# cserteGT3/RANSAC.jl

Hardware: NVIDIA B200
Metric: candidate_point_evals_per_s (higher is better)
Workload: dtype f32

## Files before the change

### ransac.jl_b200/csrc/rsc_eval.cuh

```cuda
#pragma once
#include "rsc_common.cuh"

namespace rsc {

__host__ __device__ constexpr float kappa(int type) {
  return type == RSC_PLANE ? 8.f : type == RSC_SPHERE ? 16.f : type == RSC_CYLINDER ? 16.f : 20.f;
}

__host__ __device__ constexpr float kappa_in(int type) {
  return type == RSC_PLANE ? 1.f : type == RSC_SPHERE ? 3.f : type == RSC_CYLINDER ? 3.f : 4.f;
}

__host__ __device__ inline int col_type(const rsc_cand& c) {
  if (c.type != RSC_CONE) return c.type;
  return cos(0.5 * c.p[6]) >= 0.5 ? RSC_CONE : kConeWide;
}

__device__ __forceinline__ float fmax_nan(float a, float b) {
  float r;
  asm("max.NaN.f32 %0, %1, %2;" : "=f"(r) : "f"(a), "f"(b));
  return r;
}
__device__ __forceinline__ float rsqrt_fast(float a) {
  float r;
// ... 66 lines not shown
    float wn = fmaf(wx, nx, fmaf(wy, ny, wz * nz));
    float an = fmaf(r[4], nx, fmaf(r[5], ny, r[6] * nz));
    float t1 = fmaf(r[0], an, r[9]);
    float cw = r[10] * wn;
    float nt = fmaf(rho, t1, -cw);
    return fmax_nan(e, nt);
  } else {
    float vx = fmaf(r[0], px, r[1]), vy = fmaf(r[0], py, r[2]), vz = fmaf(r[0], pz, r[3]);
    float h = fmaf(r[4], vx, fmaf(r[5], vy, r[6] * vz));
    float wx = fmaf(-r[4], h, vx), wy = fmaf(-r[5], h, vy), wz = fmaf(-r[6], h, vz);
    float ww = fmaf(wx, wx, fmaf(wy, wy, wz * wz));
    float rho = ww * rsqrt_fast(ww);
    float d = fmaf(h, r[7], -rho);
    float e = fabsf(d) + r[8];
    float wn = fmaf(wx, nx, fmaf(wy, ny, wz * nz));
    float an = fmaf(r[4], nx, fmaf(r[5], ny, r[6] * nz));
    float t1 = fmaf(r[7], an, r[9]);
    float nt = fmaf(rho, t1, -wn);
    return fmax_nan(e, nt);
  }
}

__device__ __forceinline__ float2 bc2(float s) { return make_float2(s, s); }
__device__ __forceinline__ float2 neg2(float2 a) { return make_float2(-a.x, -a.y); }
__device__ __forceinline__ float2 abs2(float2 a) { return make_float2(fabsf(a.x), fabsf(a.y)); }
__device__ __forceinline__ float2 fma2(float2 a, float2 b, float2 c) { return __ffma2_rn(a, b, c); }
__device__ __forceinline__ float2 mul2(float2 a, float2 b) { return __fmul2_rn(a, b); }
__device__ __forceinline__ float2 add2(float2 a, float2 b) { return __fadd2_rn(a, b); }
__device__ __forceinline__ float2 rsqrt2(float2 a) { return make_float2(rsqrt_fast(a.x), rsqrt_fast(a.y)); }
__device__ __forceinline__ float2 max2_nan(float2 a, float2 b) {
  return make_float2(fmax_nan(a.x, b.x), fmax_nan(a.y, b.y));
}

template <int T>
__device__ __forceinline__ float2 eval2_terms(const float2* r, float px, float py, float pz, float nx, float ny,
                                              float nz, float eps, float cosa, float2* nt_out) {
  const float2 X = bc2(px), Y = bc2(py), Z = bc2(pz), NX = bc2(nx), NY = bc2(ny), NZ = bc2(nz);
  if constexpr (T == RSC_PLANE) {
    const float2 d = fma2(r[0], X, fma2(r[1], Y, fma2(r[2], Z, r[3])));
    const float2 e = add2(abs2(d), bc2(-eps));
    const float2 nt = fma2(r[4], NX, fma2(r[5], NY, fma2(r[6], NZ, bc2(cosa))));
    *nt_out = nt;
    return e;
  } else if constexpr (T == RSC_SPHERE) {
    const float2 vx = fma2(r[0], X, r[1]), vy = fma2(r[0], Y, r[2]), vz = fma2(r[0], Z, r[3]);
    const float2 vv = fma2(vx, vx, fma2(vy, vy, mul2(vz, vz)));
    const float2 d = fma2(vv, rsqrt2(vv), r[4]);
    const float2 e = add2(abs2(d), bc2(-eps));
    const float2 s = fma2(vx, NX, fma2(vy, NY, fma2(vz, NZ, r[5])));
    const float2 nt = fma2(bc2(cosa), d, neg2(s));
    *nt_out = nt;
    return e;
  } else if constexpr (T == RSC_CYLINDER) {
    const float2 vx = fma2(r[0], X, r[1]), vy = fma2(r[0], Y, r[2]), vz = fma2(r[0], Z, r[3]);
    const float2 h = fma2(r[4], vx, fma2(r[5], vy, mul2(r[6], vz)));
    const float2 wx = fma2(neg2(r[4]), h, vx), wy = fma2(neg2(r[5]), h, vy), wz = fma2(neg2(r[6]), h, vz);
    const float2 ww = fma2(wx, wx, fma2(wy, wy, mul2(wz, wz)));
    const float2 d = fma2(ww, rsqrt2(ww), r[7]);
    const float2 e = add2(abs2(d), bc2(-eps));
    const float2 wn = fma2(wx, NX, fma2(wy, NY, fma2(wz, NZ, r[8])));
    const float2 nt = fma2(bc2(cosa), d, neg2(wn));
    *nt_out = nt;
    return e;
  } else if constexpr (T == kConeWide) {
    const float2 vx = fma2(r[0], X, r[1]), vy = fma2(r[0], Y, r[2]), vz = fma2(r[0], Z, r[3]);
    const float2 h = fma2(r[4], vx, fma2(r[5], vy, mul2(r[6], vz)));
    const float2 wx = fma2(neg2(r[4]), h, vx), wy = fma2(neg2(r[5]), h, vy), wz = fma2(neg2(r[6]), h, vz);
    const float2 ww = fma2(wx, wx, fma2(wy, wy, mul2(wz, wz)));
    const float2 rho = mul2(ww, rsqrt2(ww));
    const float2 d = fma2(neg2(rho), r[7], h);
    const float2 e = add2(abs2(d), r[8]);
    const float2 wn = fma2(wx, NX, fma2(wy, NY, mul2(wz, NZ)));
    const float2 an = fma2(r[4], NX, fma2(r[5], NY, mul2(r[6], NZ)));
    const float2 t1 = fma2(r[0], an, r[9]);
    const float2 cw = mul2(r[10], wn);
    const float2 nt = fma2(rho, t1, neg2(cw));
    *nt_out = nt;
    return e;
  } else {
    const float2 vx = fma2(r[0], X, r[1]), vy = fma2(r[0], Y, r[2]), vz = fma2(r[0], Z, r[3]);
    const float2 h = fma2(r[4], vx, fma2(r[5], vy, mul2(r[6], vz)));
    const float2 wx = fma2(neg2(r[4]), h, vx), wy = fma2(neg2(r[5]), h, vy), wz = fma2(neg2(r[6]), h, vz);
    const float2 ww = fma2(wx, wx, fma2(wy, wy, mul2(wz, wz)));
    const float2 rho = mul2(ww, rsqrt2(ww));
    const float2 d = fma2(h, r[7], neg2(rho));
    const float2 e = add2(abs2(d), r[8]);
    const float2 wn = fma2(wx, NX, fma2(wy, NY, mul2(wz, NZ)));
    const float2 an = fma2(r[4], NX, fma2(r[5], NY, mul2(r[6], NZ)));
    const float2 t1 = fma2(r[7], an, r[9]);
    const float2 nt = fma2(rho, t1, neg2(wn));
    *nt_out = nt;
    return e;
  }
}

template <int T>
__device__ __forceinline__ float2 eval2(const float2* r, float px, float py, float pz, float nx, float ny,
                                        float nz, float eps, float cosa) {
  float2 nt;
  const float2 e = eval2_terms<T>(r, px, py, pz, nx, ny, nz, eps, cosa, &nt);
  return max2_nan(e, nt);
}

template <int T>
__device__ __forceinline__ void eval2x4(const float2* r, const float* px, const float* py, const float* pz, const float* nx,
                                        const float* ny, const float* nz, float eps, float cosa, float2* m) {
#define RSC_Q for (int q = 0; q < 4; ++q)
  if constexpr (T == RSC_PLANE) {
    float2 d[4], nt[4];
#pragma unroll
    RSC_Q d[q] = fma2(r[2], bc2(pz[q]), r[3]);
#pragma unroll
    RSC_Q d[q] = fma2(r[1], bc2(py[q]), d[q]);
#pragma unroll
    RSC_Q d[q] = fma2(r[0], bc2(px[q]), d[q]);
#pragma unroll
    RSC_Q nt[q] = fma2(r[6], bc2(nz[q]), bc2(cosa));
#pragma unroll
    RSC_Q nt[q] = fma2(r[5], bc2(ny[q]), nt[q]);
#pragma unroll
    RSC_Q nt[q] = fma2(r[4], bc2(nx[q]), nt[q]);
#pragma unroll
    RSC_Q d[q] = add2(abs2(d[q]), bc2(-eps));
#pragma unroll
    RSC_Q m[q] = max2_nan(d[q], nt[q]);
  } else {
// ... 257 lines not shown
```

### ransac.jl_b200/csrc/rsc_score.cu

```cuda
#include <math.h>
#include <stdlib.h>

#include "rsc_eval.cuh"
#include "rsc_exact.cuh"

namespace rsc {

struct GroupTask {
  uint32_t cand;
  uint32_t group;
  uint32_t word;
  uint32_t slot_type;
};

struct ScoreArgs {
  PointSet ps;
  Thresh th;
  const float* rec;
  const int32_t* orig;
  const BlockTab* tab;
  int32_t cslots;
  int32_t subs_per_chunk;
  int32_t nsubs;
  int32_t* counts_valid;
  int32_t* counts_enabled;
  uint32_t* masks;
  GroupTask* wl;
  uint32_t* wl_count;
  uint32_t wl_cap;
};

constexpr int kSub = 128;
constexpr int kStages = 2;
constexpr int kSubFloats = 6 * kSub;
// ... 2 lines not shown
__device__ __forceinline__ uint32_t smem_u32(const void* p) { return (uint32_t)__cvta_generic_to_shared(p); }
__device__ __forceinline__ void mbar_init(uint64_t* bar, uint32_t count) {
  asm volatile("mbarrier.init.shared::cta.b64 [%0], %1;" ::"r"(smem_u32(bar)), "r"(count));
}
__device__ __forceinline__ void mbar_expect_tx(uint64_t* bar, uint32_t bytes) {
  asm volatile("mbarrier.arrive.expect_tx.shared::cta.b64 _, [%0], %1;" ::"r"(smem_u32(bar)), "r"(bytes) : "memory");
}
__device__ __forceinline__ void mbar_wait(uint64_t* bar, uint32_t parity) {
  asm volatile(
      "{\n"
      ".reg .pred p;\n"
      "WAIT_%=:\n"
      "mbarrier.try_wait.parity.shared::cta.b64 p, [%0], %1;\n"
      "@p bra DONE_%=;\n"
      "bra WAIT_%=;\n"
      "DONE_%=:\n"
      "}\n" ::"r"(smem_u32(bar)),
      "r"(parity)
      : "memory");
}
__device__ __forceinline__ void bulk_g2s(void* dst, const void* src, uint32_t bytes, uint64_t* bar) {
  asm volatile("cp.async.bulk.shared::cluster.global.mbarrier::complete_tx::bytes [%0], [%1], %2, [%3];" ::"r"(
                   smem_u32(dst)),
               "l"(src), "r"(bytes), "r"(smem_u32(bar))
               : "memory");
}

__device__ __forceinline__ void issue_subtile(const float* src, int64_t stride, float* stage, uint64_t* bar) {
  mbar_expect_tx(bar, kSubBytes);
#pragma unroll
  for (int f = 0; f < 6; ++f) bulk_g2s(stage + f * kSub, src + f * stride, kSub * 4, bar);
}

template <int T, int K, int U, bool MASKS>
__device__ __forceinline__ void score_body(const ScoreArgs& a, int slot0, float* wstage, uint64_t* wbar) {
  constexpr int NR = RecN<T>::n;
  constexpr bool kPacked = (K % 2 == 0) && U < 5;
  constexpr int KP = kPacked ? K / 2 : 1;
  constexpr bool kOrderJQ = (U == 3);
  float r[kPacked ? 1 : K][NR];
  float2 r2[KP][NR];
  float band[K];
  int cnte[K], cntv[K];
  const int tid = threadIdx.x, lane = tid & 31;
  const float* recp = a.rec + slot0 + tid;
#pragma unroll
  for (int k = 0; k < K; ++k) {
#pragma unroll
    for (int f = 0; f < NR; ++f) {
      const float v = recp[(size_t)f * a.cslots + k * kThreads];
      if constexpr (kPacked) {
        if (k & 1)
          r2[k / 2][f].y = v;
        else
          r2[k / 2][f].x = v;
      } else {
        r[k][f] = v;
      }
    }
    band[k] = recp[(size_t)kBandField * a.cslots + k * kThreads];
    cnte[k] = 0;
    cntv[k] = 0;
  }
  constexpr int PT = public_type(T);
  const float eps = a.th.eps[PT], cosa = a.th.cosa[PT];
  const bool honour = (a.th.honour_enabled >> PT) & 1u;

  const int sub0 = blockIdx.y * a.subs_per_chunk;
  const int nsub = min(a.subs_per_chunk, a.nsubs - sub0);
  const uint32_t* enp = a.ps.enabled + (size_t)sub0 * (kSub / 32);
  const uint32_t* vap = a.ps.valid + (size_t)sub0 * (kSub / 32);
  uint32_t* maskp = MASKS ? a.masks + (size_t)sub0 * (kSub / 32) * a.cslots + slot0 + tid : nullptr;
  const int64_t stride = a.ps.y - a.ps.x;
  const float* src0 = a.ps.x + (int64_t)sub0 * kSub;
  if (lane == 0) {
#pragma unroll
    for (int s = 0; s < kStages; ++s)
      if (s < nsub) issue_subtile(src0 + s * kSub, stride, wstage + s * kSubFloats, wbar + s);
  }

  auto body4 = [&](const float* gp, uint32_t (&mask)[K], float (&mabs)[K]) {
    const float4 X = *reinterpret_cast<const float4*>(gp);
    const float4 Y = *reinterpret_cast<const float4*>(gp + kSub);
    const float4 Z = *reinterpret_cast<const float4*>(gp + 2 * kSub);
    const float4 U4 = *reinterpret_cast<const float4*>(gp + 3 * kSub);
    const float4 V = *reinterpret_cast<const float4*>(gp + 4 * kSub);
    const float4 W = *reinterpret_cast<const float4*>(gp + 5 * kSub);
    const float px[4] = {X.x, X.y, X.z, X.w}, py[4] = {Y.x, Y.y, Y.z, Y.w}, pz[4] = {Z.x, Z.y, Z.z, Z.w};
    const float nx[4] = {U4.x, U4.y, U4.z, U4.w}, ny[4] = {V.x, V.y, V.z, V.w}, nz[4] = {W.x, W.y, W.z, W.w};
    if constexpr (kPacked && U == 4) {
#pragma unroll
      for (int j = 0; j < KP; ++j) {
        float2 m[4];
        eval2x4<T>(r2[j], px, py, pz, nx, ny, nz, eps, cosa, m);
#pragma unroll
        for (int q = 0; q < 4; ++q) {
          mask[2 * j] = __funnelshift_l(__float_as_uint(m[q].x), mask[2 * j], 1);
          mask[2 * j + 1] = __funnelshift_l(__float_as_uint(m[q].y), mask[2 * j + 1], 1);
          mabs[2 * j] = fmin_nan(mabs[2 * j], fabsf(m[q].x));
          mabs[2 * j + 1] = fmin_nan(mabs[2 * j + 1], fabsf(m[q].y));
        }
      }
      return;
    }
    if constexpr (kPacked && kOrderJQ) {
#pragma unroll
      for (int j = 0; j < KP; ++j) {
        float2 m[4];
#pragma unroll
        for (int q = 0; q < 4; ++q) m[q] = eval2<T>(r2[j], px[q], py[q], pz[q], nx[q], ny[q], nz[q], eps, cosa);
#pragma unroll
        for (int q = 0; q < 4; ++q) {
          mask[2 * j] = __funnelshift_l(__float_as_uint(m[q].x), mask[2 * j], 1);
          mask[2 * j + 1] = __funnelshift_l(__float_as_uint(m[q].y), mask[2 * j + 1], 1);
          mabs[2 * j] = fmin_nan(mabs[2 * j], fabsf(m[q].x));
          mabs[2 * j + 1] = fmin_nan(mabs[2 * j + 1], fabsf(m[q].y));
        }
      }
      return;
    }
    if constexpr (!kPacked && U == 6) {
#pragma unroll
      for (int k = 0; k < K; ++k) {
        float m[4];
#pragma unroll
        for (int q = 0; q < 4; ++q) m[q] = eval<T>(r[k], px[q], py[q], pz[q], nx[q], ny[q], nz[q], eps, cosa);
#pragma unroll
        for (int q = 0; q < 4; ++q) {
          mask[k] = __funnelshift_l(__float_as_uint(m[q]), mask[k], 1);
          mabs[k] = fmin_nan(mabs[k], fabsf(m[q]));
        }
      }
      return;
    }
#pragma unroll
    for (int q = 0; q < 4; ++q) {
      if constexpr (kPacked) {
// ... 31 lines not shown
    if constexpr (MASKS) {
      const uint32_t gate = honour ? en : va;
#pragma unroll
      for (int k = 0; k < K; ++k) maskp[(size_t)gi * a.cslots + k * kThreads] = __brev(mask[k]) & gate;
    }
    if (amb && va) {
      const int64_t gw = (int64_t)sub0 * (kSub / 32) + gi;
#pragma unroll
      for (int k = 0; k < K; ++k) {
        if (mabs[k] > band[k]) continue;
        const int slot = slot0 + k * kThreads + tid;
        const int o = a.orig[slot];
        if (o < 0) continue;
        const uint32_t pos = atomicAdd(a.wl_count, 1u);
        if (pos < a.wl_cap) a.wl[pos] = GroupTask{(uint32_t)o, (uint32_t)gw, __brev(mask[k]), (uint32_t)slot | ((uint32_t)T << 28)};
      }
    }
  };

  for (int it = 0; it < nsub; ++it) {
    const int st = it % kStages;
    mbar_wait(wbar + st, (it / kStages) & 1);
    const float* sx = wstage + st * kSubFloats;
#pragma unroll 1
    for (int g = 0; g < kSub / 32; ++g) {
      uint32_t mask[K];
      float mabs[K];
#pragma unroll
      for (int k = 0; k < K; ++k) {
        mask[k] = 0u;
        mabs[k] = __int_as_float(0x7f800000);
      }
      const float* gx = sx + g * 32;
#pragma unroll(U >= 3 ? 1 : U)
      for (int i4 = 0; i4 < 32; i4 += 4) body4(gx + i4, mask, mabs);
      const int gi = it * (kSub / 32) + g;
      epilogue(mask, mabs, gi, __ldg(enp + gi), __ldg(vap + gi));
    }
    __syncwarp();
    if (lane == 0 && it + kStages < nsub) issue_subtile(src0 + (it + kStages) * kSub, stride, wstage + st * kSubFloats, wbar + st);
  }
#pragma unroll
  for (int k = 0; k < K; ++k) {
    const int o = a.orig[slot0 + k * kThreads + tid];
    if (o >= 0) {
      if (cnte[k]) atomicAdd(a.counts_enabled + o, cnte[k]);
      if (!honour && cntv[k]) atomicAdd(a.counts_valid + o, cntv[k]);
    }
  }
}

template <int T, int K, int MINB, int U, bool MASKS>
__global__ void __launch_bounds__(kThreads, MINB) score_kernel(const __grid_constant__ ScoreArgs a) {
  __shared__ __align__(128) float stages[kThreads / 32][kStages * kSubFloats];
  __shared__ __align__(8) uint64_t bars[kThreads / 32][kStages];
  const BlockTab bt = a.tab[blockIdx.x];
  if (bt.type != T) return;
  const int warp = threadIdx.x >> 5;
  if ((threadIdx.x & 31) == 0) {
#pragma unroll
    for (int s = 0; s < kStages; ++s) mbar_init(&bars[warp][s], 1);
    asm volatile("fence.mbarrier_init.release.cluster;" ::: "memory");
  }
  __syncwarp();
  score_body<T, K, U, MASKS>(a, bt.slot0, stages[warp], bars[warp]);
}

template <int K, int MINB, bool MASKS>
__global__ void __launch_bounds__(kThreads, MINB) score_kernel_any(const __grid_constant__ ScoreArgs a) {
  __shared__ __align__(128) float stages[kThreads / 32][kStages * kSubFloats];
  __shared__ __align__(8) uint64_t bars[kThreads / 32][kStages];
  const BlockTab bt = a.tab[blockIdx.x];
  if (bt.type < 0) return;
  const int warp = threadIdx.x >> 5;
  if ((threadIdx.x & 31) == 0) {
#pragma unroll
    for (int s = 0; s < kStages; ++s) mbar_init(&bars[warp][s], 1);
    asm volatile("fence.mbarrier_init.release.cluster;" ::: "memory");
  }
  __syncwarp();
  switch (bt.type) {
    case RSC_PLANE:
      score_body<RSC_PLANE, K, 1, MASKS>(a, bt.slot0, stages[warp], bars[warp]);
      break;
    case RSC_SPHERE:
      score_body<RSC_SPHERE, K, 1, MASKS>(a, bt.slot0, stages[warp], bars[warp]);
      break;
    case RSC_CYLINDER:
      score_body<RSC_CYLINDER, K, 1, MASKS>(a, bt.slot0, stages[warp], bars[warp]);
      break;
    case RSC_CONE:
      score_body<RSC_CONE, K, 1, MASKS>(a, bt.slot0, stages[warp], bars[warp]);
      break;
    default:
      score_body<kConeWide, K, 1, MASKS>(a, bt.slot0, stages[warp], bars[warp]);
      break;
  }
}
// ... 77 lines not shown
    const bool used = pr.cand_bit >> 31;
    const rsc_cand c = cands[cand];
    ex::ConeTrig tr{1.0, 0.0};
    if (c.type == RSC_CONE) {
      if (trig) {
        tr = trig[cand];
      } else {
        tr.ct = cos(-c.p[6] / 2);
        tr.st = sin(-c.p[6] / 2);
      }
    }
    const uint32_t pt = pr.point;
    ex::V3 P, N;
    ex::point64(a.ps, pt, &P, &N);
    const bool ok = ex::compat(c, tr, a.th, P, N);
    if (ok != used) apply_flip(a, cand, c.type, slot_of[cand], pt, ok);
  }
}

__global__ void select_counts_kernel(const rsc_cand* __restrict__ cands, int C,
                                     const int32_t* __restrict__ cv, const int32_t* __restrict__ ce,
                                     uint32_t honour_enabled, int32_t* __restrict__ out) {
  const int i = blockIdx.x * blockDim.x + threadIdx.x;
  if (i >= C) return;
  const int t = cands[i].type;
  const bool honour = (t >= 0 && t < RSC_NTYPES) ? ((honour_enabled >> t) & 1u) : true;
  out[i] = honour ? ce[i] : cv[i];
}

struct ColSlots {
  int v[kColTypes];
};

__global__ void __launch_bounds__(1024) compile_kernel(const rsc_cand* __restrict__ cands, int C, const Thresh th,
                                                       const ColSlots spcs, int cslots,
                                                       int ncols, float pmax, float nmax,
                                                       const uint32_t* __restrict__ d_bounds,
                                                       float* __restrict__ rec, int32_t* __restrict__ orig,
                                                       int32_t* __restrict__ slot_of,
                                                       BlockTab* __restrict__ tab) {
  __shared__ int cnt[kColTypes], off[kColTypes], run[kColTypes], tot[kColTypes];
  __shared__ int wcnt[kColTypes][32], woff[kColTypes][32];
  const int tid = threadIdx.x, lane = tid & 31, warp = tid >> 5;
  if (d_bounds) {
    pmax = sqrtf(__uint_as_float(d_bounds[0])) * 1.000001f;
    nmax = sqrtf(__uint_as_float(d_bounds[1])) * 1.000001f;
  }
  if (tid < kColTypes) {
    cnt[tid] = 0;
    run[tid] = 0;
  }
  __syncthreads();
  for (int i = tid; i < C; i += blockDim.x) {
    const int t = cands[i].type;
    if (t >= 0 && t < RSC_NTYPES) atomicAdd(&cnt[col_type(cands[i])], 1);
  }
  __syncthreads();
  if (tid == 0) {
    const int order[kColTypes] = {kConeWide, RSC_CONE, RSC_CYLINDER, RSC_SPHERE, RSC_PLANE};
    int s = 0, col = 0;
    for (int oi = 0; oi < kColTypes; ++oi) {
      const int t = order[oi];
      off[t] = s;
      const int spc = spcs.v[t];
      const int nb = (cnt[t] + spc - 1) / spc;
      for (int b = 0; b < nb && col < ncols; ++b) tab[col++] = BlockTab{t, s + b * spc};
      s += nb * spc;
    }
    for (; col < ncols; ++col) tab[col] = BlockTab{-1, 0};
  }
  __syncthreads();
  for (int base = 0; base < C; base += blockDim.x) {
    const int i = base + tid;
    int t = -1;
    if (i < C) {
      t = cands[i].type;
      t = (t < 0 || t >= RSC_NTYPES) ? -1 : col_type(cands[i]);
    }
    int myrank = 0;
#pragma unroll
    for (int tt = 0; tt < kColTypes; ++tt) {
      const unsigned b = __ballot_sync(0xffffffffu, t == tt);
      if (t == tt) myrank = __popc(b & ((1u << lane) - 1u));
      if (lane == 0) wcnt[tt][warp] = __popc(b);
    }
    __syncthreads();
    if (warp == 0) {
#pragma unroll
      for (int tt = 0; tt < kColTypes; ++tt) {
        const int v = wcnt[tt][lane];
        int inc = v;
#pragma unroll
        for (int d = 1; d < 32; d <<= 1) {
          const int o = __shfl_up_sync(0xffffffffu, inc, d);
          if (lane >= d) inc += o;
        }
        woff[tt][lane] = inc - v;
        if (lane == 31) tot[tt] = inc;
      }
    }
    __syncthreads();
    if (i < C) {
      if (t >= 0) {
        const int slot = off[t] + run[t] + woff[t][warp] + myrank;
        float r[kRecFields];
        compile_record(cands[i], t, th, pmax, nmax, r);
#pragma unroll
        for (int f = 0; f < kRecFields; ++f) rec[(size_t)f * cslots + slot] = r[f];
        orig[slot] = i;
        slot_of[i] = slot;
      } else {
        slot_of[i] = -1;
      }
    }
    __syncthreads();
    if (tid < kColTypes) run[tid] += tot[tid];
    __syncthreads();
  }
  for (int t = 0; t < kColTypes; ++t) {
    const int n = cnt[t];
    if (n == 0) continue;
    const int spc = spcs.v[t];
    const int padded = ((n + spc - 1) / spc) * spc;
    const int src = off[t] + n - 1;
    for (int s = n + tid; s < padded; s += blockDim.x) {
      const int dst = off[t] + s;
#pragma unroll
      for (int f = 0; f < kRecFields; ++f) rec[(size_t)f * cslots + dst] = rec[(size_t)f * cslots + src];
      orig[dst] = -1;
    }
  }
}

__global__ void __launch_bounds__(1024) masks_transpose_kernel(const uint32_t* __restrict__ gm,
                                                               const int32_t* __restrict__ slot_of,
                                                               int C, int cslots, int64_t words,
                                                               uint32_t* __restrict__ out) {
  __shared__ uint32_t t[32][33];
  const int c0 = blockIdx.x * 32;
  const int64_t g0 = (int64_t)blockIdx.y * 32;
  {
    const int c = c0 + threadIdx.x;
    const int64_t g = g0 + threadIdx.y;
    uint32_t v = 0;
    if (c < C && g < words) {
      const int s = slot_of[c];
      if (s >= 0) v = gm[(size_t)g * cslots + s];
    }
    t[threadIdx.y][threadIdx.x] = v;
  }
  __syncthreads();
  {
    const int c = c0 + threadIdx.y;
    const int64_t g = g0 + threadIdx.x;
    if (c < C && g < words) out[(size_t)c * words + g] = t[threadIdx.x][threadIdx.y];
  }
}

Thresh make_thresh(const rsc_params* p) {
  Thresh th;
  for (int t = 0; t < RSC_NTYPES; ++t) {
    th.eps_d[t] = p->eps[t];
    th.cosa_d[t] = cos(p->alpha[t]);
    th.eps[t] = (float)th.eps_d[t];
    th.cosa[t] = (float)th.cosa_d[t];
  }
  th.honour_enabled = 0xFu;
  if (p->compat_flags & RSC_COMPAT_SPHERE_IGNORES_ENABLED) th.honour_enabled &= ~(1u << RSC_SPHERE);
  return th;
}

using ScoreFn = void (*)(const ScoreArgs);
struct Tiling {
  int K, minb, U;
  ScoreFn fn[kColTypes];
  ScoreFn fn_masks[kColTypes];
};
#define RSC_TILING(K, MINB, U)                                                                          \
  Tiling {                                                                                              \
    K, MINB, U,                                                                                         \
        {score_kernel<RSC_PLANE, K, MINB, U, false>, score_kernel<RSC_SPHERE, K, MINB, U, false>,       \
         score_kernel<RSC_CYLINDER, K, MINB, U, false>, score_kernel<RSC_CONE, K, MINB, U, false>,      \
         score_kernel<kConeWide, K, MINB, U, false>},                                                   \
    {                                                                                                   \
      score_kernel<RSC_PLANE, K, MINB, U, true>, score_kernel<RSC_SPHERE, K, MINB, U, true>,            \
          score_kernel<RSC_CYLINDER, K, MINB, U, true>, score_kernel<RSC_CONE, K, MINB, U, true>,       \
          score_kernel<kConeWide, K, MINB, U, true>                                                     \
    }                                                                                                   \
  }
#ifdef RSC_EXP_K
static const Tiling kTilings[] = {RSC_TILING(1, 4, 1), RSC_TILING(RSC_EXP_K, RSC_EXP_MINB, RSC_EXP_U)};
#else
static const Tiling kTilings[] = {
    RSC_TILING(1, 4, 1), RSC_TILING(2, 4, 1), RSC_TILING(4, 3, 1), RSC_TILING(4, 4, 1), RSC_TILING(8, 2, 1), RSC_TILING(4, 4, 3), RSC_TILING(4, 3, 3),
    RSC_TILING(4, 4, 5), RSC_TILING(4, 3, 5), RSC_TILING(4, 4, 6), RSC_TILING(4, 3, 6), RSC_TILING(8, 2, 5),
};
#endif
static const Tiling* find_tiling(int K, int minb, int U) {
  for (const Tiling& t : kTilings)
    if (t.K == K && t.minb == minb && t.U == U) return &t;
  return nullptr;
}

static int cap_k(int C) { return C >= 3072 ? 8 : (C >= 768 ? 2 : 1); }

static const Tiling* pick_tiling(int type, int C) {
  static const char* names[kColTypes] = {"RSC_CFG_PLANE", "RSC_CFG_SPHERE", "RSC_CFG_CYLINDER", "RSC_CFG_CONE", "RSC_CFG_CONE"};
  static const int dflt[kColTypes][3] = {{4, 4, 3}, {4, 3, 3}, {4, 3, 3}, {4, 3, 3}, {4, 3, 3}};
  int K = dflt[type][0], minb = dflt[type][1], U = dflt[type][2];
  if (const char* e = getenv(names[type])) {
    int a = 0, b = 0, c = 0;
    if (sscanf(e, "%d,%d,%d", &a, &b, &c) == 3 && find_tiling(a, b, c)) K = a, minb = b, U = c;
  }
  const int kc = cap_k(C);
  if (K > kc) {
    K = kc;
    minb = 4, U = 1;
  }
  return find_tiling(K, minb, U);
}

// ... 35 lines not shown
    return RSC_OK;
  }
  if (ps.n_pad >= ((int64_t)1 << 32)) return fail(ctx, RSC_E_ARG, "point set too large for one shard (>= 2^32)");
  {
    const int64_t sd = ps.y - ps.x;
    if (ps.z - ps.y != sd || ps.nx - ps.z != sd || ps.ny - ps.nx != sd || ps.nz - ps.ny != sd)
      return fail(ctx, RSC_E_ARG, "score: the six SoA rows of the point set must be equally spaced");
  }
  const SlotLayout L = slot_layout(C);
  const int ncols = L.ncols, cslots = L.cslots;
  ctx->last_cslots = cslots;
  const int nsubs = (int)(ps.n_pad / kSub);
  const int64_t groups = ps.n_pad / 32;

  RSC_CUDA(ctx, ctx->rec.ensure((size_t)kRecFields * cslots * sizeof(float)));
  RSC_CUDA(ctx, ctx->orig.ensure((size_t)cslots * sizeof(int32_t)));
  RSC_CUDA(ctx, ctx->slot_of.ensure((size_t)C * sizeof(int32_t)));
  RSC_CUDA(ctx, ctx->blktab.ensure((size_t)ncols * sizeof(BlockTab)));
  RSC_CUDA(ctx, ctx->counts.ensure((size_t)2 * C * sizeof(int32_t)));
  RSC_CUDA(ctx, ctx->worklist.ensure(ctx->wl_cap * sizeof(GroupTask)));
  RSC_CUDA(ctx, ctx->wl_count.ensure(16));
  if (want_masks) RSC_CUDA(ctx, ctx->masks_gm.ensure((size_t)groups * cslots * sizeof(uint32_t)));

  int32_t* cv = d_counts_valid ? d_counts_valid : ctx->counts.as<int32_t>();
  int32_t* ce = d_counts_enabled ? d_counts_enabled : ctx->counts.as<int32_t>() + C;
  if (!accumulate) {
    RSC_CUDA(ctx, cudaMemsetAsync(cv, 0, (size_t)C * sizeof(int32_t), st));
    RSC_CUDA(ctx, cudaMemsetAsync(ce, 0, (size_t)C * sizeof(int32_t), st));
  }
  RSC_CUDA(ctx, ctx->pairs.ensure(ctx->wl_cap * 8));
  RSC_CUDA(ctx, cudaMemsetAsync(ctx->wl_count.p, 0, 2 * sizeof(uint32_t), st));

  if (cloud->exact() && !ps.xyz64) return fail(ctx, RSC_E_STATE, "score: a point set of an exact cloud lacks its float64 coordinates");
  Thresh thx = th;
  thx.exact_in = cloud->exact();
  compile_kernel<<<1, 1024, 0, st>>>(d_cands, C, thx, L.spcs, cslots, ncols, cloud->pmax, cloud->nmax, d_bounds,
                                     ctx->rec.as<float>(), ctx->orig.as<int32_t>(),
                                     ctx->slot_of.as<int32_t>(), ctx->blktab.as<BlockTab>());
  RSC_CUDA(ctx, cudaGetLastError());

  ScoreArgs a;
  a.ps = ps;
  a.th = thx;
  a.rec = ctx->rec.as<float>();
  a.orig = ctx->orig.as<int32_t>();
  a.tab = ctx->blktab.as<BlockTab>();
  a.cslots = cslots;
  a.nsubs = nsubs;
  a.counts_valid = cv;
  a.counts_enabled = ce;
  a.masks = want_masks ? ctx->masks_gm.as<uint32_t>() : nullptr;
  a.wl = ctx->worklist.as<GroupTask>();
  a.wl_count = ctx->wl_count.as<uint32_t>();
  a.wl_cap = (uint32_t)ctx->wl_cap;

  const int waves = getenv("RSC_WAVES") ? atoi(getenv("RSC_WAVES")) : 32;
  const int est_cols = (C + kThreads * 4 - 1) / (kThreads * 4);
  const long target = (long)ctx->sm_count * 4 * waves;
  long chunks = (target + est_cols - 1) / est_cols;
  if (chunks > nsubs) chunks = nsubs;
  if (chunks < 1) chunks = 1;
  if (chunks > 65535) chunks = 65535;
  a.subs_per_chunk = (int)((nsubs + chunks - 1) / chunks);
  chunks = (nsubs + a.subs_per_chunk - 1) / a.subs_per_chunk;
  dim3 grid((unsigned)ncols, (unsigned)chunks);
  static const double fork_min = getenv("RSC_FORK_MIN") ? atof(getenv("RSC_FORK_MIN")) : 1e9;
  const bool fork = (double)C * (double)ps.n_pad >= fork_min && !getenv("RSC_NOFORK");

  RSC_CUDA(ctx, cudaEventRecord(ctx->evk0, st));
  const int K0 = L.til[0]->K;
  bool uniform_k = K0 <= 2;
  for (int t = 1; t < kColTypes; ++t) uniform_k = uniform_k && L.til[t]->K == K0;
  if (!fork && uniform_k && !getenv("RSC_NOFUSE")) {
    if (K0 == 1) {
      if (want_masks)
        score_kernel_any<1, 4, true><<<grid, kThreads, 0, st>>>(a);
      else
        score_kernel_any<1, 4, false><<<grid, kThreads, 0, st>>>(a);
    } else {
      if (want_masks)
        score_kernel_any<2, 4, true><<<grid, kThreads, 0, st>>>(a);
      else
        score_kernel_any<2, 4, false><<<grid, kThreads, 0, st>>>(a);
    }
    RSC_CUDA(ctx, cudaGetLastError());
  } else {
    if (fork) RSC_CUDA(ctx, cudaEventRecord(ctx->ev_fork, st));
    const int order[kColTypes] = {RSC_CONE, kConeWide, RSC_CYLINDER, RSC_SPHERE, RSC_PLANE};
    for (int oi = 0; oi < kColTypes; ++oi) {
      const int t = order[oi];
      cudaStream_t s = st;
      if (fork && oi > 0) {
        s = ctx->sfork[oi - 1];
        RSC_CUDA(ctx, cudaStreamWaitEvent(s, ctx->ev_fork, 0));
      }
      (want_masks ? L.til[t]->fn_masks[t] : L.til[t]->fn[t])<<<grid, kThreads, 0, s>>>(a);
      RSC_CUDA(ctx, cudaGetLastError());
      if (fork && oi > 0) {
        RSC_CUDA(ctx, cudaEventRecord(ctx->ev_join[oi - 1], s));
        RSC_CUDA(ctx, cudaStreamWaitEvent(st, ctx->ev_join[oi - 1], 0));
      }
    }
  }
  RSC_CUDA(ctx, cudaGetLastError());
  RSC_CUDA(ctx, cudaEventRecord(ctx->evk1, st));
  ctx->stats.score_launches += 1;
  ctx->stats.evals += (int64_t)C * ps.n;
  ctx->stats.cands_scored += C;

  fixup_scan_kernel<<<ctx->sm_count * 8, 256, 0, st>>>(a, d_cands, ctx->slot_of.as<int32_t>(), ctx->pairs.as<AmbPair>(),
                                                       ctx->wl_count.as<uint32_t>() + 1, (uint32_t)ctx->wl_cap);
  RSC_CUDA(ctx, cudaGetLastError());
  fixup_pair_kernel<<<ctx->sm_count * 4, 256, 0, st>>>(a, d_cands, reinterpret_cast<const ex::ConeTrig*>(d_trig),
                                                       ctx->slot_of.as<int32_t>(), ctx->pairs.as<AmbPair>(),
                                                       ctx->wl_count.as<uint32_t>() + 1, (uint32_t)ctx->wl_cap);
  RSC_CUDA(ctx, cudaGetLastError());
  if (d_counts_policy) {
    select_counts_kernel<<<(C + 255) / 256, 256, 0, st>>>(d_cands, C, cv, ce, th.honour_enabled, d_counts_policy);
    RSC_CUDA(ctx, cudaGetLastError());
  }
  return RSC_OK;
}

__global__ void audit_compile_kernel(const rsc_cand* __restrict__ cands, int C, const Thresh th, float pmax, float nmax,
                                     float* __restrict__ rec , int32_t* __restrict__ cols) {
  const int i = blockIdx.x * blockDim.x + threadIdx.x;
  if (i >= C) return;
  const int col = (cands[i].type < 0 || cands[i].type >= RSC_NTYPES) ? RSC_PLANE : col_type(cands[i]);
  float r[kRecFields];
// ... 78 lines not shown
```

Baseline: 1578.

## Skip normal-angle term when distance rejects whole warp, sort candidates spatially

```diff
diff --git a/ransac.jl_b200/csrc/rsc_eval.cuh b/ransac.jl_b200/csrc/rsc_eval.cuh
--- a/ransac.jl_b200/csrc/rsc_eval.cuh
+++ b/ransac.jl_b200/csrc/rsc_eval.cuh
@@ -122,66 +122,72 @@
   return make_float2(fmax_nan(a.x, b.x), fmax_nan(a.y, b.y));
 }
 
-template <int T>
-__device__ __forceinline__ float2 eval2_terms(const float2* r, float px, float py, float pz, float nx, float ny,
-                                              float nz, float eps, float cosa, float2* nt_out) {
-  const float2 X = bc2(px), Y = bc2(py), Z = bc2(pz), NX = bc2(nx), NY = bc2(ny), NZ = bc2(nz);
+struct Mid2 {
+  float2 x, y, z, s;
+};
+
+template <int T>
+__device__ __forceinline__ float2 eval2_dist(const float2* r, float px, float py, float pz, float eps, Mid2* md) {
+  const float2 X = bc2(px), Y = bc2(py), Z = bc2(pz);
   if constexpr (T == RSC_PLANE) {
     const float2 d = fma2(r[0], X, fma2(r[1], Y, fma2(r[2], Z, r[3])));
-    const float2 e = add2(abs2(d), bc2(-eps));
-    const float2 nt = fma2(r[4], NX, fma2(r[5], NY, fma2(r[6], NZ, bc2(cosa))));
-    *nt_out = nt;
-    return e;
+    return add2(abs2(d), bc2(-eps));
   } else if constexpr (T == RSC_SPHERE) {
     const float2 vx = fma2(r[0], X, r[1]), vy = fma2(r[0], Y, r[2]), vz = fma2(r[0], Z, r[3]);
     const float2 vv = fma2(vx, vx, fma2(vy, vy, mul2(vz, vz)));
     const float2 d = fma2(vv, rsqrt2(vv), r[4]);
-    const float2 e = add2(abs2(d), bc2(-eps));
-    const float2 s = fma2(vx, NX, fma2(vy, NY, fma2(vz, NZ, r[5])));
-    const float2 nt = fma2(bc2(cosa), d, neg2(s));
-    *nt_out = nt;
-    return e;
-  } else if constexpr (T == RSC_CYLINDER) {
-    const float2 vx = fma2(r[0], X, r[1]), vy = fma2(r[0], Y, r[2]), vz = fma2(r[0], Z, r[3]);
-    const float2 h = fma2(r[4], vx, fma2(r[5], vy, mul2(r[6], vz)));
-    const float2 wx = fma2(neg2(r[4]), h, vx), wy = fma2(neg2(r[5]), h, vy), wz = fma2(neg2(r[6]), h, vz);
-    const float2 ww = fma2(wx, wx, fma2(wy, wy, mul2(wz, wz)));
-    const float2 d = fma2(ww, rsqrt2(ww), r[7]);
-    const float2 e = add2(abs2(d), bc2(-eps));
-    const float2 wn = fma2(wx, NX, fma2(wy, NY, fma2(wz, NZ, r[8])));
-    const float2 nt = fma2(bc2(cosa), d, neg2(wn));
-    *nt_out = nt;
-    return e;
-  } else if constexpr (T == kConeWide) {
-    const float2 vx = fma2(r[0], X, r[1]), vy = fma2(r[0], Y, r[2]), vz = fma2(r[0], Z, r[3]);
-    const float2 h = fma2(r[4], vx, fma2(r[5], vy, mul2(r[6], vz)));
-    const float2 wx = fma2(neg2(r[4]), h, vx), wy = fma2(neg2(r[5]), h, vy), wz = fma2(neg2(r[6]), h, vz);
-    const float2 ww = fma2(wx, wx, fma2(wy, wy, mul2(wz, wz)));
-    const float2 rho = mul2(ww, rsqrt2(ww));
-    const float2 d = fma2(neg2(rho), r[7], h);
-    const float2 e = add2(abs2(d), r[8]);
-    const float2 wn = fma2(wx, NX, fma2(wy, NY, mul2(wz, NZ)));
-    const float2 an = fma2(r[4], NX, fma2(r[5], NY, mul2(r[6], NZ)));
-    const float2 t1 = fma2(r[0], an, r[9]);
-    const float2 cw = mul2(r[10], wn);
-    const float2 nt = fma2(rho, t1, neg2(cw));
-    *nt_out = nt;
-    return e;
+    *md = Mid2{vx, vy, vz, d};
+    return add2(abs2(d), bc2(-eps));
   } else {
     const float2 vx = fma2(r[0], X, r[1]), vy = fma2(r[0], Y, r[2]), vz = fma2(r[0], Z, r[3]);
     const float2 h = fma2(r[4], vx, fma2(r[5], vy, mul2(r[6], vz)));
     const float2 wx = fma2(neg2(r[4]), h, vx), wy = fma2(neg2(r[5]), h, vy), wz = fma2(neg2(r[6]), h, vz);
     const float2 ww = fma2(wx, wx, fma2(wy, wy, mul2(wz, wz)));
-    const float2 rho = mul2(ww, rsqrt2(ww));
-    const float2 d = fma2(h, r[7], neg2(rho));
-    const float2 e = add2(abs2(d), r[8]);
-    const float2 wn = fma2(wx, NX, fma2(wy, NY, mul2(wz, NZ)));
+    if constexpr (T == RSC_CYLINDER) {
+      const float2 d = fma2(ww, rsqrt2(ww), r[7]);
+      *md = Mid2{wx, wy, wz, d};
+      return add2(abs2(d), bc2(-eps));
+    } else {
+      const float2 rho = mul2(ww, rsqrt2(ww));
+      *md = Mid2{wx, wy, wz, rho};
+      const float2 d = (T == kConeWide) ? fma2(neg2(rho), r[7], h) : fma2(h, r[7], neg2(rho));
+      return add2(abs2(d), r[8]);
+    }
+  }
+}
+
+template <int T>
+__device__ __forceinline__ float2 eval2_angle(const float2* r, const Mid2& md, float nx, float ny, float nz, float cosa) {
+  const float2 NX = bc2(nx), NY = bc2(ny), NZ = bc2(nz);
+  if constexpr (T == RSC_PLANE) {
+    return fma2(r[4], NX, fma2(r[5], NY, fma2(r[6], NZ, bc2(cosa))));
+  } else if constexpr (T == RSC_SPHERE) {
+    const float2 s = fma2(md.x, NX, fma2(md.y, NY, fma2(md.z, NZ, r[5])));
+    return fma2(bc2(cosa), md.s, neg2(s));
+  } else if constexpr (T == RSC_CYLINDER) {
+    const float2 wn = fma2(md.x, NX, fma2(md.y, NY, fma2(md.z, NZ, r[8])));
+    return fma2(bc2(cosa), md.s, neg2(wn));
+  } else if constexpr (T == kConeWide) {
+    const float2 wn = fma2(md.x, NX, fma2(md.y, NY, mul2(md.z, NZ)));
+    const float2 an = fma2(r[4], NX, fma2(r[5], NY, mul2(r[6], NZ)));
+    const float2 t1 = fma2(r[0], an, r[9]);
+    const float2 cw = mul2(r[10], wn);
+    return fma2(md.s, t1, neg2(cw));
+  } else {
+    const float2 wn = fma2(md.x, NX, fma2(md.y, NY, mul2(md.z, NZ)));
     const float2 an = fma2(r[4], NX, fma2(r[5], NY, mul2(r[6], NZ)));
     const float2 t1 = fma2(r[7], an, r[9]);
-    const float2 nt = fma2(rho, t1, neg2(wn));
-    *nt_out = nt;
-    return e;
-  }
+    return fma2(md.s, t1, neg2(wn));
+  }
+}
+
+template <int T>
+__device__ __forceinline__ float2 eval2_terms(const float2* r, float px, float py, float pz, float nx, float ny,
+                                              float nz, float eps, float cosa, float2* nt_out) {
+  Mid2 md;
+  const float2 e = eval2_dist<T>(r, px, py, pz, eps, &md);
+  *nt_out = eval2_angle<T>(r, md, nx, ny, nz, cosa);
+  return e;
 }
 
 template <int T>
diff --git a/ransac.jl_b200/csrc/rsc_score.cu b/ransac.jl_b200/csrc/rsc_score.cu
--- a/ransac.jl_b200/csrc/rsc_score.cu
+++ b/ransac.jl_b200/csrc/rsc_score.cu
@@ -1,5 +1,7 @@
 #include <math.h>
 #include <stdlib.h>
+
+#include <cub/block/block_radix_sort.cuh>
 
 #include "rsc_eval.cuh"
 #include "rsc_exact.cuh"
@@ -68,12 +70,14 @@
   for (int f = 0; f < 6; ++f) bulk_g2s(stage + f * kSub, src + f * stride, kSub * 4, bar);
 }
 
-template <int T, int K, int U, bool MASKS>
+template <int T, int K, int U, bool MASKS, bool SPLIT = false>
 __device__ __forceinline__ void score_body(const ScoreArgs& a, int slot0, float* wstage, uint64_t* wbar) {
   constexpr int NR = RecN<T>::n;
   constexpr bool kPacked = (K % 2 == 0) && U < 5;
   constexpr int KP = kPacked ? K / 2 : 1;
   constexpr bool kOrderJQ = (U == 3);
+  constexpr bool kSplit = SPLIT && kPacked && kOrderJQ;
+  constexpr float kNBound = 1152921504606846976.f;
   float r[kPacked ? 1 : K][NR];
   float2 r2[KP][NR];
   float band[K];
@@ -98,6 +102,14 @@
     cnte[k] = 0;
     cntv[k] = 0;
   }
+  bool lane_full = false;
+  if constexpr (kSplit && T == RSC_PLANE) {
+#pragma unroll
+    for (int j = 0; j < KP; ++j) {
+      lane_full |= !(fabsf(r2[j][4].x) + fabsf(r2[j][5].x) + fabsf(r2[j][6].x) <= kNBound);
+      lane_full |= !(fabsf(r2[j][4].y) + fabsf(r2[j][5].y) + fabsf(r2[j][6].y) <= kNBound);
+    }
+  }
   constexpr int PT = public_type(T);
   const float eps = a.th.eps[PT], cosa = a.th.cosa[PT];
   const bool honour = (a.th.honour_enabled >> PT) & 1u;
@@ -115,7 +127,7 @@
       if (s < nsub) issue_subtile(src0 + s * kSub, stride, wstage + s * kSubFloats, wbar + s);
   }
 
-  auto body4 = [&](const float* gp, uint32_t (&mask)[K], float (&mabs)[K]) {
+  auto body4 = [&](const float* gp, uint32_t (&mask)[K], float (&mabs)[K], bool full) {
     const float4 X = *reinterpret_cast<const float4*>(gp);
     const float4 Y = *reinterpret_cast<const float4*>(gp + kSub);
     const float4 Z = *reinterpret_cast<const float4*>(gp + 2 * kSub);
@@ -139,6 +151,31 @@
       }
       return;
     }
+    if constexpr (kSplit) {
+#pragma unroll
+      for (int q = 0; q < 4; ++q) {
+        float2 m[KP];
+        Mid2 md[KP];
+        bool need = full;
+#pragma unroll
+        for (int j = 0; j < KP; ++j) {
+          m[j] = eval2_dist<T>(r2[j], px[q], py[q], pz[q], eps, &md[j]);
+          need |= !(m[j].x > band[2 * j]) | !(m[j].y > band[2 * j + 1]);
+        }
+        if (__any_sync(0xffffffffu, need)) {
+#pragma unroll
+          for (int j = 0; j < KP; ++j) m[j] = max2_nan(m[j], eval2_angle<T>(r2[j], md[j], nx[q], ny[q], nz[q], cosa));
+        }
+#pragma unroll
+        for (int j = 0; j < KP; ++j) {
+          mask[2 * j] = __funnelshift_l(__float_as_uint(m[j].x), mask[2 * j], 1);
+          mask[2 * j + 1] = __funnelshift_l(__float_as_uint(m[j].y), mask[2 * j + 1], 1);
+          mabs[2 * j] = fmin_nan(mabs[2 * j], fabsf(m[j].x));
+          mabs[2 * j + 1] = fmin_nan(mabs[2 * j + 1], fabsf(m[j].y));
+        }
+      }
+      return;
+    }
     if constexpr (kPacked && kOrderJQ) {
 #pragma unroll
       for (int j = 0; j < KP; ++j) {
@@ -236,8 +273,13 @@
         mabs[k] = __int_as_float(0x7f800000);
       }
       const float* gx = sx + g * 32;
+      bool full = lane_full;
+      if constexpr (kSplit) {
+        const float sn = fabsf(gx[3 * kSub + lane]) + fabsf(gx[4 * kSub + lane]) + fabsf(gx[5 * kSub + lane]);
+        full |= __any_sync(0xffffffffu, !(sn <= kNBound));
+      }
 #pragma unroll(U >= 3 ? 1 : U)
-      for (int i4 = 0; i4 < 32; i4 += 4) body4(gx + i4, mask, mabs);
+      for (int i4 = 0; i4 < 32; i4 += 4) body4(gx + i4, mask, mabs, full);
       const int gi = it * (kSub / 32) + g;
       epilogue(mask, mabs, gi, __ldg(enp + gi), __ldg(vap + gi));
     }
@@ -254,7 +296,7 @@
   }
 }
 
-template <int T, int K, int MINB, int U, bool MASKS>
+template <int T, int K, int MINB, int U, bool MASKS, bool SPLIT>
 __global__ void __launch_bounds__(kThreads, MINB) score_kernel(const __grid_constant__ ScoreArgs a) {
   __shared__ __align__(128) float stages[kThreads / 32][kStages * kSubFloats];
   __shared__ __align__(8) uint64_t bars[kThreads / 32][kStages];
@@ -267,7 +309,7 @@
     asm volatile("fence.mbarrier_init.release.cluster;" ::: "memory");
   }
   __syncwarp();
-  score_body<T, K, U, MASKS>(a, bt.slot0, stages[warp], bars[warp]);
+  score_body<T, K, U, MASKS, SPLIT>(a, bt.slot0, stages[warp], bars[warp]);
 }
 
 template <int K, int MINB, bool MASKS>
@@ -411,6 +453,66 @@
   int v[kColTypes];
 };
 
+constexpr int kSortItems = 8;
+constexpr int kSortMax = 1024 * kSortItems;
+__device__ __forceinline__ int col_order(int oi) {
+  return oi == 0 ? kConeWide : oi == 1 ? RSC_CONE : oi == 2 ? RSC_CYLINDER : oi == 3 ? RSC_SPHERE : RSC_PLANE;
+}
+
+__device__ __forceinline__ uint32_t spread3(uint32_t v) {
+  v &= 0x1ffu;
+  v = (v | (v << 16)) & 0x030000ffu;
+  v = (v | (v << 8)) & 0x0300f00fu;
+  v = (v | (v << 4)) & 0x030c30c3u;
+  v = (v | (v << 2)) & 0x09249249u;
+  return v;
+}
+__device__ __forceinline__ uint32_t quant(float x, float lo, float inv, int cells) {
+  const float f = (x - lo) * inv;
+  return f >= 0.f ? (uint32_t)fminf(f, (float)(cells - 1)) : 0u;
+}
+__device__ __forceinline__ unsigned f2ord(float f) {
+  const unsigned u = __float_as_uint(f);
+  return (u & 0x80000000u) ? ~u : (u | 0x80000000u);
+}
+__device__ __forceinline__ float ord2f(unsigned u) { return __uint_as_float((u & 0x80000000u) ? (u & 0x7fffffffu) : ~u); }
+
+__device__ __forceinline__ int warp_slot(int p, int spc) {
+  const int K = spc / kThreads, u = p % spc, w = u / (32 * K), v = u % (32 * K);
+  return (p - u) + (v / 32) * kThreads + w * 32 + (v % 32);
+}
+
+__device__ __forceinline__ void anchor(const rsc_cand& c, float* a) {
+  const int o = c.type == RSC_CYLINDER ? 3 : 0;
+  for (int i = 0; i < 3; ++i) a[i] = (float)c.p[o + i];
+}
+
+__device__ inline uint32_t loc_key(const rsc_cand& c, const float* lo, const float* inv, const float* c0) {
+  float q[3] = {(float)c.p[0], (float)c.p[1], (float)c.p[2]};
+  if (c.type == RSC_CYLINDER || c.type == RSC_PLANE) {
+    const int ob = c.type == RSC_CYLINDER ? 3 : 0, oa = c.type == RSC_CYLINDER ? 0 : 3;
+    const float b[3] = {(float)c.p[ob], (float)c.p[ob + 1], (float)c.p[ob + 2]};
+    const float ax[3] = {(float)c.p[oa], (float)c.p[oa + 1], (float)c.p[oa + 2]};
+    const float aa = ax[0] * ax[0] + ax[1] * ax[1] + ax[2] * ax[2];
+    const float ad = ax[0] * (c0[0] - b[0]) + ax[1] * (c0[1] - b[1]) + ax[2] * (c0[2] - b[2]);
+    float t = aa > 0.f ? ad / aa : 0.f;
+    if (!isfinite(t)) t = 0.f;
+    for (int i = 0; i < 3; ++i)
+      q[i] = c.type == RSC_CYLINDER ? b[i] + ax[i] * t : c0[i] - ax[i] * t;
+    if (c.type == RSC_PLANE) {
+      const float s = (ax[2] < 0.f || (ax[2] == 0.f && (ax[1] < 0.f || (ax[1] == 0.f && ax[0] < 0.f)))) ? -1.f : 1.f;
+      const float il = aa > 0.f ? s * rsqrtf(aa) : 0.f;
+      const uint32_t hx = quant(ax[0] * il, -1.f, 4.f, 8), hy = quant(ax[1] * il, -1.f, 4.f, 8);
+      const uint32_t m = spread3(quant(q[0], lo[0], inv[0] * 0.25f, 128)) | (spread3(quant(q[1], lo[1], inv[1] * 0.25f, 128)) << 1) |
+                         (spread3(quant(q[2], lo[2], inv[2] * 0.25f, 128)) << 2);
+      return (hx << 24) | (hy << 21) | m;
+    }
+  }
+  return spread3(quant(q[0], lo[0], inv[0], 512)) | (spread3(quant(q[1], lo[1], inv[1], 512)) << 1) |
+         (spread3(quant(q[2], lo[2], inv[2], 512)) << 2);
+}
+
+template <bool SORT>
 __global__ void __launch_bounds__(1024) compile_kernel(const rsc_cand* __restrict__ cands, int C, const Thresh th,
                                                        const ColSlots spcs, int cslots,
                                                        int ncols, float pmax, float nmax,
@@ -420,6 +522,7 @@
                                                        BlockTab* __restrict__ tab) {
   __shared__ int cnt[kColTypes], off[kColTypes], run[kColTypes], tot[kColTypes];
   __shared__ int wcnt[kColTypes][32], woff[kColTypes][32];
+  __shared__ unsigned blo[3], bhi[3];
   const int tid = threadIdx.x, lane = tid & 31, warp = tid >> 5;
   if (d_bounds) {
     pmax = sqrtf(__uint_as_float(d_bounds[0])) * 1.000001f;
@@ -429,17 +532,33 @@
     cnt[tid] = 0;
     run[tid] = 0;
   }
+  if (SORT && tid < 3) {
+    blo[tid] = f2ord(pmax);
+    bhi[tid] = f2ord(-pmax);
+  }
   __syncthreads();
+  float alo[3] = {pmax, pmax, pmax}, ahi[3] = {-pmax, -pmax, -pmax};
   for (int i = tid; i < C; i += blockDim.x) {
     const int t = cands[i].type;
     if (t >= 0 && t < RSC_NTYPES) atomicAdd(&cnt[col_type(cands[i])], 1);
+    if (SORT && t >= 0 && t < RSC_NTYPES) {
+      float a[3];
+      anchor(cands[i], a);
+      for (int d = 0; d < 3; ++d)
+        if (isfinite(a[d])) alo[d] = fminf(alo[d], fmaxf(a[d], -pmax)), ahi[d] = fmaxf(ahi[d], fminf(a[d], pmax));
+    }
+  }
+  if constexpr (SORT) {
+    for (int d = 0; d < 3; ++d) {
+      atomicMin(&blo[d], f2ord(alo[d]));
+      atomicMax(&bhi[d], f2ord(ahi[d]));
+    }
   }
   __syncthreads();
   if (tid == 0) {
-    const int order[kColTypes] = {kConeWide, RSC_CONE, RSC_CYLINDER, RSC_SPHERE, RSC_PLANE};
     int s = 0, col = 0;
     for (int oi = 0; oi < kColTypes; ++oi) {
-      const int t = order[oi];
+      const int t = col_order(oi);
       off[t] = s;
       const int spc = spcs.v[t];
       const int nb = (cnt[t] + spc - 1) / spc;
@@ -449,7 +568,59 @@
     for (; col < ncols; ++col) tab[col] = BlockTab{-1, 0};
   }
   __syncthreads();
-  for (int base = 0; base < C; base += blockDim.x) {
+  if constexpr (SORT) {
+    float lo[3], inv[3], c0[3];
+    for (int d = 0; d < 3; ++d) {
+      lo[d] = ord2f(blo[d]);
+      const float hi = ord2f(bhi[d]);
+      const float w = hi - lo[d];
+      inv[d] = w > 0.f ? 512.f / w : 0.f;
+      c0[d] = 0.5f * (lo[d] + hi);
+    }
+    uint32_t key[kSortItems];
+    int32_t val[kSortItems];
+#pragma unroll
+    for (int j = 0; j < kSortItems; ++j) {
+      const int i = tid * kSortItems + j;
+      key[j] = 0xffffffffu;
+      val[j] = i;
+      if (i < C) {
+        const int t = cands[i].type;
+        if (t >= 0 && t < RSC_NTYPES) {
+          const int ct = col_type(cands[i]);
+          int rank = 0;
+          for (int oi = 0; oi < kColTypes; ++oi)
+            if (col_order(oi) == ct) rank = oi;
+          key[j] = ((uint32_t)rank << 27) | loc_key(cands[i], lo, inv, c0);
+        } else {
+          slot_of[i] = -1;
+        }
+      }
+    }
+    using Sort = cub::BlockRadixSort<uint32_t, 1024, kSortItems, int32_t>;
+    __shared__ typename Sort::TempStorage sort_tmp;
+    Sort(sort_tmp).Sort(key, val, 0, 30);
+#pragma unroll
+    for (int j = 0; j < kSortItems; ++j) {
+      if (key[j] == 0xffffffffu) continue;
+      const int i = val[j], pos = tid * kSortItems + j;
+      const int rank = (int)(key[j] >> 27), t = col_order(rank);
+      int before = 0;
+      for (int oi = 0; oi < rank; ++oi) before += cnt[col_order(oi)];
+      slot_of[i] = off[t] + warp_slot(pos - before, spcs.v[t]);
+    }
+    __syncthreads();
+    for (int i = tid; i < C; i += blockDim.x) {
+      const int slot = slot_of[i];
+      if (slot < 0) continue;
+      float r[kRecFields];
+      compile_record(cands[i], col_type(cands[i]), th, pmax, nmax, r);
+#pragma unroll
+      for (int f = 0; f < kRecFields; ++f) rec[(size_t)f * cslots + slot] = r[f];
+      orig[slot] = i;
+    }
+  }
+  for (int base = 0; base < C && !SORT; base += blockDim.x) {
     const int i = base + tid;
     int t = -1;
     if (i < C) {
@@ -496,14 +667,15 @@
     if (tid < kColTypes) run[tid] += tot[tid];
     __syncthreads();
   }
+  if constexpr (SORT) __syncthreads();
   for (int t = 0; t < kColTypes; ++t) {
     const int n = cnt[t];
     if (n == 0) continue;
     const int spc = spcs.v[t];
     const int padded = ((n + spc - 1) / spc) * spc;
-    const int src = off[t] + n - 1;
+    const int src = off[t] + (SORT ? warp_slot(n - 1, spc) : n - 1);
     for (int s = n + tid; s < padded; s += blockDim.x) {
-      const int dst = off[t] + s;
+      const int dst = off[t] + (SORT ? warp_slot(s, spc) : s);
 #pragma unroll
       for (int f = 0; f < kRecFields; ++f) rec[(size_t)f * cslots + dst] = rec[(size_t)f * cslots + src];
       orig[dst] = -1;
@@ -554,18 +726,19 @@
   int K, minb, U;
   ScoreFn fn[kColTypes];
   ScoreFn fn_masks[kColTypes];
+  ScoreFn fn_split[kColTypes];
+  ScoreFn fn_masks_split[kColTypes];
 };
-#define RSC_TILING(K, MINB, U)                                                                          \
-  Tiling {                                                                                              \
-    K, MINB, U,                                                                                         \
-        {score_kernel<RSC_PLANE, K, MINB, U, false>, score_kernel<RSC_SPHERE, K, MINB, U, false>,       \
-         score_kernel<RSC_CYLINDER, K, MINB, U, false>, score_kernel<RSC_CONE, K, MINB, U, false>,      \
-         score_kernel<kConeWide, K, MINB, U, false>},                                                   \
-    {                                                                                                   \
-      score_kernel<RSC_PLANE, K, MINB, U, true>, score_kernel<RSC_SPHERE, K, MINB, U, true>,            \
-          score_kernel<RSC_CYLINDER, K, MINB, U, true>, score_kernel<RSC_CONE, K, MINB, U, true>,       \
-          score_kernel<kConeWide, K, MINB, U, true>                                                     \
-    }                                                                                                   \
+#define RSC_TILING_FNS(K, MINB, U, MASKS, SPLIT)                                                                     \
+  {                                                                                                                   \
+    score_kernel<RSC_PLANE, K, MINB, U, MASKS, SPLIT>, score_kernel<RSC_SPHERE, K, MINB, U, MASKS, SPLIT>,            \
+        score_kernel<RSC_CYLINDER, K, MINB, U, MASKS, SPLIT>, score_kernel<RSC_CONE, K, MINB, U, MASKS, SPLIT>,       \
+        score_kernel<kConeWide, K, MINB, U, MASKS, SPLIT>                                                             \
+  }
+#define RSC_TILING(K, MINB, U)                                                                                        \
+  Tiling {                                                                                                            \
+    K, MINB, U, RSC_TILING_FNS(K, MINB, U, false, false), RSC_TILING_FNS(K, MINB, U, true, false),                    \
+        RSC_TILING_FNS(K, MINB, U, false, (U == 3)), RSC_TILING_FNS(K, MINB, U, true, (U == 3))                       \
   }
 #ifdef RSC_EXP_K
 static const Tiling kTilings[] = {RSC_TILING(1, 4, 1), RSC_TILING(RSC_EXP_K, RSC_EXP_MINB, RSC_EXP_U)};
@@ -667,11 +840,23 @@
   RSC_CUDA(ctx, cudaMemsetAsync(ctx->wl_count.p, 0, 2 * sizeof(uint32_t), st));
 
   if (cloud->exact() && !ps.xyz64) return fail(ctx, RSC_E_STATE, "score: a point set of an exact cloud lacks its float64 coordinates");
+  static const double fork_min = getenv("RSC_FORK_MIN") ? atof(getenv("RSC_FORK_MIN")) : 1e9;
+  const bool fork = (double)C * (double)ps.n_pad >= fork_min && !getenv("RSC_NOFORK");
+  const int K0 = L.til[0]->K;
+  bool uniform_k = K0 <= 2;
+  for (int t = 1; t < kColTypes; ++t) uniform_k = uniform_k && L.til[t]->K == K0;
+  const bool fused = !fork && uniform_k && !getenv("RSC_NOFUSE");
+  const char* split_env = getenv("RSC_SCORE_SPLIT");
+  const bool split = !(split_env && atoi(split_env) == 0);
+  bool split_kernels = false;
+  for (int t = 0; t < kColTypes; ++t) split_kernels = split_kernels || (L.til[t]->U == 3 && L.til[t]->K % 2 == 0);
+  const bool sort = split && !fused && split_kernels && C <= kSortMax;
+
   Thresh thx = th;
   thx.exact_in = cloud->exact();
-  compile_kernel<<<1, 1024, 0, st>>>(d_cands, C, thx, L.spcs, cslots, ncols, cloud->pmax, cloud->nmax, d_bounds,
-                                     ctx->rec.as<float>(), ctx->orig.as<int32_t>(),
-                                     ctx->slot_of.as<int32_t>(), ctx->blktab.as<BlockTab>());
+  (sort ? compile_kernel<true> : compile_kernel<false>)<<<1, 1024, 0, st>>>(
+      d_cands, C, thx, L.spcs, cslots, ncols, cloud->pmax, cloud->nmax, d_bounds, ctx->rec.as<float>(), ctx->orig.as<int32_t>(),
+      ctx->slot_of.as<int32_t>(), ctx->blktab.as<BlockTab>());
   RSC_CUDA(ctx, cudaGetLastError());
 
   ScoreArgs a;
@@ -699,14 +884,9 @@
   a.subs_per_chunk = (int)((nsubs + chunks - 1) / chunks);
   chunks = (nsubs + a.subs_per_chunk - 1) / a.subs_per_chunk;
   dim3 grid((unsigned)ncols, (unsigned)chunks);
-  static const double fork_min = getenv("RSC_FORK_MIN") ? atof(getenv("RSC_FORK_MIN")) : 1e9;
-  const bool fork = (double)C * (double)ps.n_pad >= fork_min && !getenv("RSC_NOFORK");
 
   RSC_CUDA(ctx, cudaEventRecord(ctx->evk0, st));
-  const int K0 = L.til[0]->K;
-  bool uniform_k = K0 <= 2;
-  for (int t = 1; t < kColTypes; ++t) uniform_k = uniform_k && L.til[t]->K == K0;
-  if (!fork && uniform_k && !getenv("RSC_NOFUSE")) {
+  if (fused) {
     if (K0 == 1) {
       if (want_masks)
         score_kernel_any<1, 4, true><<<grid, kThreads, 0, st>>>(a);
@@ -729,7 +909,8 @@
         s = ctx->sfork[oi - 1];
         RSC_CUDA(ctx, cudaStreamWaitEvent(s, ctx->ev_fork, 0));
       }
-      (want_masks ? L.til[t]->fn_masks[t] : L.til[t]->fn[t])<<<grid, kThreads, 0, s>>>(a);
+      const Tiling& tl = *L.til[t];
+      (split ? (want_masks ? tl.fn_masks_split[t] : tl.fn_split[t]) : (want_masks ? tl.fn_masks[t] : tl.fn[t]))<<<grid, kThreads, 0, s>>>(a);
       RSC_CUDA(ctx, cudaGetLastError());
       if (fork && oi > 0) {
         RSC_CUDA(ctx, cudaEventRecord(ctx->ev_join[oi - 1], s));
```

New measurement: 1651, median of 6. 1.05x the previous value.
